# Kudo510/ImageSequenceRegistrationfor6DPoseEstimationLabeling

Measured on AMD Instinct MI355X. Metric: registered images/sec (T-LESS obj 1-like, synthetic) + final Chamfer error, higher is better.
Workload: dtype bf16

## Files before the change

imagesequenceregistrationfor6dposeestimationlabeling_amd/_capi.py:

```python
from __future__ import annotations

import ctypes as C
from pathlib import Path

import torch

import os

_PKG = Path(__file__).resolve().parent
LIB_PATH = Path(os.environ["ISR_HIP_LIB"]) if os.environ.get("ISR_HIP_LIB") else _PKG / "libisr_hip.so"

ISR_OK = 0
ABI_VERSION = 6
DTYPE_BF16 = 0
DTYPE_F32 = 1
DTYPE_BF16_LOG2 = 2
DTYPE_BF16_LOG2_SCREENED = 3
RANSAC_STAGED = 0
RANSAC_SEQUENTIAL = 1
INLIERS_REFIT = 0
INLIERS_RANSAC = 1
FINAL_REFIT = 0
FINAL_EPNP = 1
TUNE = {"nn_path": 0, "nn_filter": 1, "icp_warm": 2, "nn_plan_rq": 3, "nn_plan_blocks": 4,
        "nn_tile_st": 5, "nn_tile_sq": 6, "nn_tile_tb": 7, "ep_wsum_valu": 8, "k1_f32_chain": 9, "k1_split": 10}


class IsrError(RuntimeError):
    pass


_lib = None

_vp = C.c_void_p
_i = C.c_int
_sz = C.c_size_t
_d = C.c_double
_f = C.c_float
_u64 = C.c_uint64
_i64 = C.c_int64

SIGNATURES = {
    "isr_abi_version": (_i, []),
    "isr_last_error": (C.c_char_p, []),
    "isr_device_count": (_i, []),
    "isr_tuning_set": (_i, [_i, _i]),
    "isr_tuning_get": (_i, [_i]),
    "isr_corr_argmax_workspace_bytes": (_sz, [_i, _i, _i, _i]),
# ... 91 lines not shown
DENSITY_SIGNATURES = {
    "isr_density_pack_bytes": (_sz, [_i, _vp, _i]),
    "isr_density_pack": (_i, [_i, _vp, _i, _vp, _f, _vp, _vp, _vp, _sz]),
    "isr_density_eval": (_i, [_vp, _sz, _i, _vp, _i, _vp, _i, _vp, _vp]),
    "isr_density_march": (_i, [_vp, _sz, _i, _vp, _i, _vp, _vp, _vp, _i, _i, _f, _vp, _vp, _vp, _vp, _vp, _vp]),
    "isr_density_eval_host": (_i, [_vp, _sz, _i, _vp, _i, _vp, _i, _vp]),
    "isr_density_march_host": (_i, [_vp, _sz, _i, _vp, _i, _vp, _vp, _vp, _i, _i, _f, _vp, _vp, _vp, _vp, _vp]),
    "isr_density_sincos_host": (_i, [_vp, _sz, _vp, _vp]),
    "isr_density_activations_host": (_i, [_vp, _sz, _f, _vp, _vp]),
}

DENSITY_DIR_SIGNATURES = {
    "isr_density_march_dir": (_i, [_vp, _sz, _i, _vp, _i, _vp, _vp, _vp, _i, _i, _f, _i, _vp, _vp, _vp, _vp, _vp, _vp]),
    "isr_density_march_dir_host": (_i, [_vp, _sz, _i, _vp, _i, _vp, _vp, _vp, _i, _i, _f, _i, _vp, _vp, _vp, _vp, _vp]),
    "isr_density_march_given_host": (_i, [_vp, _vp, _i, _i, _f, _i, _vp, _vp, _vp]),
}

RADIUS_SIGNATURES = {
    "isr_radius_workspace_bytes": (_sz, [_i]),
    "isr_radius_count": (_i, [_vp, _i, _d, _i, _vp, _vp, _sz, _vp]),
    "isr_radius_count_host": (_i, [_vp, _i, _d, _i, _vp]),
}

KNN_SIGNATURES = {
    "isr_knn_workspace_bytes": (_sz, [_i, _i, _i]),
    "isr_knn": (_i, [_vp, _i, _vp, _i, _i, _vp, _vp, _vp, _sz, _vp]),
    "isr_knn_host": (_i, [_vp, _i, _vp, _i, _i, _vp, _vp]),
    "isr_local_frames": (_i, [_vp, _i, _vp, _i, _i, _vp, _vp, _vp]),
    "isr_local_frames_host": (_i, [_vp, _i, _vp, _i, _i, _vp, _vp]),
}

_RAYS_SPEC = [_i, _vp, _vp, _vp, _vp, _i, _i, _i, _i, _i, _f, _f, _f, _f, _f, _f, _i, _u64]
RAYS_SIGNATURES = {
    "isr_rays_workspace_bytes": (_sz, [_i, _i]),
    "isr_rays_bundle": (_i, [*_RAYS_SPEC, _vp, _vp, _vp, _vp, _vp]),
    "isr_rays_bundle_host": (_i, [*_RAYS_SPEC, _vp, _vp, _vp, _vp]),
    "isr_rays_select_count": (_i, [*_RAYS_SPEC, _vp, _i, _i, _vp, _vp, _sz, _vp]),
    "isr_rays_select_emit": (_i, [*_RAYS_SPEC, _vp, _i, _i, _vp, _sz, _i64, _vp, _vp, _vp, _vp, _vp, _vp]),
    "isr_rays_select_count_host": (_i, [*_RAYS_SPEC, _vp, _i, _i, _vp]),
    "isr_rays_select_emit_host": (_i, [*_RAYS_SPEC, _vp, _i, _i, _i64, _vp, _vp, _vp, _vp, _vp]),
    "isr_sample_nearest": (_i, [_vp, _i, _i, _i, _i, _vp, _i, _vp, _vp]),
    "isr_sample_nearest_host": (_i, [_vp, _i, _i, _i, _i, _vp, _i, _vp]),
    "isr_rays_philox_host": (_i, [_vp, _vp, _vp, _vp]),
}

_RADIANCE_FIELD = [_vp, _sz, _i, _vp, _i, _i, _i]
# ... 144 lines not shown
    "isr_seq_refit_sums_host": (_i, [_vp, _vp, _vp, _vp, _vp, _vp, _i, _i, _i, _d, _vp, _vp, _vp]),
}


def lib() -> C.CDLL:
    global _lib
    if _lib is not None:
        return _lib
    if not LIB_PATH.exists():
        raise IsrError(
            f"{LIB_PATH} is missing: build it with "
            "`python -m imagesequenceregistrationfor6dposeestimationlabeling_amd.build` "
            "(there is no CPU fallback)")
    try:
        L = C.CDLL(str(LIB_PATH))
    except OSError as e:
        raise IsrError(f"cannot load {LIB_PATH}: {e}") from e
    for name, (res, args) in {**SIGNATURES, **FIELD_SIGNATURES, **FPS_SIGNATURES, **DENSITY_SIGNATURES,
                               **DENSITY_DIR_SIGNATURES, **RADIUS_SIGNATURES, **MC_SIGNATURES, **KNN_SIGNATURES,
                               **RAYS_SIGNATURES, **RADIANCE_SIGNATURES, **RESAMPLE_SIGNATURES,
                               **CONTRASTIVE_SIGNATURES, **FIELD_GRAD_SIGNATURES, **SAMPLE_GRAD_SIGNATURES,
                               **EA_GRAD_SIGNATURES, **RADIANCE_GRAD_SIGNATURES, **AUGMENT_SIGNATURES,
                               **ADAM_SIGNATURES, **RAY_LOSSES_SIGNATURES, **COLOR_AUG_SIGNATURES, **INGEST_SIGNATURES,
                               **ICP_PLANE_SIGNATURES, **SEQ_REFIT_SIGNATURES}.items():
        try:
            fn = getattr(L, name)
        except AttributeError as e:
            raise IsrError(f"{LIB_PATH} does not export {name}") from e
        fn.restype = res
        fn.argtypes = args
    if L.isr_abi_version() != ABI_VERSION:
        raise IsrError(f"ABI version {L.isr_abi_version()} != {ABI_VERSION}")
    _lib = L
    return L


def check(rc: int, what: str) -> None:
    if rc != ISR_OK:
        msg = lib().isr_last_error()
        raise IsrError(f"{what} failed ({rc}): {msg.decode() if msg else ''}")


def ptr(t) -> int | None:
    if t is None:
        return None
    return t.data_ptr()

# ... 22 lines not shown
```

imagesequenceregistrationfor6dposeestimationlabeling_amd/csrc/capi_common.hip:

```cpp
#include "isr_common.hpp"

#include <atomic>
#include <cstdlib>
#include <cstring>

namespace isr {

char* last_error_buf() {
  static thread_local char buf[512] = {0};
  return buf;
}

void set_error(const char* fmt, ...) {
  va_list ap;
  va_start(ap, fmt);
  vsnprintf(last_error_buf(), 512, fmt, ap);
  va_end(ap);
}

namespace {

struct Tuning {
  std::atomic<int> v[ISR_TUNE_COUNT];
  Tuning() {
    const int defaults[ISR_TUNE_COUNT] = {-1, -1, 1, 0, 0, 0, 0, 0, 0, 0, 0};
    for (int i = 0; i < ISR_TUNE_COUNT; ++i) v[i].store(defaults[i], std::memory_order_relaxed);
    if (const char* e = getenv("ISR_NN_GRID")) { if (e[0] >= '0' && e[0] <= '2') v[ISR_TUNE_NN_PATH] = e[0] - '0'; }
    if (const char* e = getenv("ISR_NN_FILTER")) { if (e[0] == '0' || e[0] == '1') v[ISR_TUNE_NN_FILTER] = e[0] - '0'; }
    if (const char* e = getenv("ISR_ICP_WARM")) { if (e[0] == '0') v[ISR_TUNE_ICP_WARM] = 0; }
    if (const char* e = getenv("ISR_NN_PLAN")) {
      int rq = 0; long want = 0;
      if (sscanf(e, "%d,%ld", &rq, &want) >= 1) {
        if (rq == 1 || rq == 4) v[ISR_TUNE_NN_PLAN_RQ] = rq;
        if (want > 0) v[ISR_TUNE_NN_PLAN_BLOCKS] = (int)want;
      }
    }
    if (const char* e = getenv("ISR_NN_TILE")) {
      double st = 0, sq = 0; int tb = 0;
      (void)sscanf(e, "%lf,%lf,%d", &st, &sq, &tb);
      if (st > 0) v[ISR_TUNE_NN_TILE_ST] = (int)(st * 1000.0 + 0.5);
      if (sq > 0) v[ISR_TUNE_NN_TILE_SQ] = (int)(sq * 1000.0 + 0.5);
      if (tb > 0) v[ISR_TUNE_NN_TILE_TB] = tb;
    }
  }
};

Tuning& tuning_state() {
  static Tuning t;
  return t;
}

const int tuning_loaded = (tuning_state(), 0);
// ... 85 lines not shown
```

imagesequenceregistrationfor6dposeestimationlabeling_amd/csrc/nn_batched.hip:

```cpp
#include "block_prims.hpp"
#include "isr_common.hpp"

#include <cstddef>
#include <cstdlib>

namespace {

#ifndef ISR_NN_PACKED_BATCH
#define ISR_NN_PACKED_BATCH 1
#endif
constexpr int kThreads = 256;
constexpr int kTile = 256;
constexpr int kGroup = 8;
constexpr int kNV = 18;

__device__ __forceinline__ void xform64(const double* __restrict__ T, float x, float y, float z,
                                        double& ox, double& oy, double& oz) {
  if (T == nullptr) {
    ox = x; oy = y; oz = z;
    return;
  }
  const double dx = x, dy = y, dz = z;
  ox = fma(T[2], dz, fma(T[1], dy, fma(T[0], dx, T[3])));
  oy = fma(T[6], dz, fma(T[5], dy, fma(T[4], dx, T[7])));
  oz = fma(T[10], dz, fma(T[9], dy, fma(T[8], dx, T[11])));
}

constexpr int kUnresolved = -2;

template <int RQ>
__device__ __forceinline__ int query_of(int r) {
  return (int)blockIdx.x * RQ * kThreads + ((int)threadIdx.x >> 6) * (RQ * 64) + r * 64 + ((int)threadIdx.x & 63);
}

__global__ __launch_bounds__(256) void tile_box_kernel(const float* __restrict__ tgt, int Nt, float* __restrict__ box) {
  __shared__ float red[6][4];
  const int j = blockIdx.x * 256 + threadIdx.x;
  float v[6] = {3.0e38f, 3.0e38f, 3.0e38f, -3.0e38f, -3.0e38f, -3.0e38f};
  if (j < Nt) {
#pragma unroll
    for (int a = 0; a < 3; ++a) v[a] = v[3 + a] = tgt[3 * (size_t)j + a];
  }
#pragma unroll
  for (int a = 0; a < 3; ++a) {
#pragma unroll
    for (int o = 32; o >= 1; o >>= 1) {
      v[a] = fminf(v[a], __shfl_xor(v[a], o, 64));
      v[3 + a] = fmaxf(v[3 + a], __shfl_xor(v[3 + a], o, 64));
    }
  }
  if ((threadIdx.x & 63) == 0) {
// ... 846 lines not shown
      launch_search(p, grid, stream, qry, Nq, tgt, Nt, tq, tt, packed ? nullptr : part_d2, packed ? nullptr : part_idx, nullptr, unres,
                    packed, nullptr);
    ISR_CHECK_LAUNCH("nn_search_kernel");
    const dim3 fgrid(p.fblocks, nb);
    if (cov)
      nn_finalize_kernel<true><<<fgrid, kThreads, 0, stream>>>(qry, Nq, tgt, Tq, Tt, p.nsplit,
                                                               radius, part_d2, part_idx, b0,
                                                               nn_idx, nn_d, part_sums, nullptr, packed);
    else
      nn_finalize_kernel<false><<<fgrid, kThreads, 0, stream>>>(qry, Nq, tgt, Tq, Tt, p.nsplit,
                                                                radius, part_d2, part_idx, b0,
                                                                nn_idx, nn_d, part_sums, nullptr, packed);
    ISR_CHECK_LAUNCH("nn_finalize_kernel");
  }
  if (sum_d || sum_d2 || n_in || cov) {
    const dim3 rblock(32, 8);
    nn_reduce_kernel<<<(B + 7) / 8, rblock, 0, stream>>>(part_sums, p.fblocks, B, sum_d, sum_d2,
                                                         n_in, cov);
    ISR_CHECK_LAUNCH("nn_reduce_kernel");
  }
  return ISR_OK;
}

extern "C" int isr_add_metric(const float* verts, int V, const double* Ta, const double* Tb, int B,
                              double* mean_out, isr_stream_t stream) {
  ISR_REQUIRE(verts && mean_out, "isr_add_metric: null pointer");
  ISR_REQUIRE(V > 0 && B > 0, "isr_add_metric: V=%d B=%d", V, B);
  add_metric_kernel<<<B, kThreads, 0, isr::as_stream(stream)>>>(verts, V, Ta, Tb, mean_out);
  ISR_CHECK_LAUNCH("add_metric_kernel");
  return ISR_OK;
}

extern "C" size_t isr_icp_workspace_bytes(int Ns, int Nt) {
  if (Ns <= 0 || Nt <= 0) return 0;
  const NNPlan p = make_plan(Ns, Nt, 1, true);
  return isr::align_up((size_t)p.fblocks * kNV * sizeof(double), 256) + isr::align_up((size_t)Ns * 8, 256) +
         2 * isr::align_up((size_t)Ns * 4, 256) + isr::align_up((size_t)((Nt + kTile - 1) / kTile) * 6 * sizeof(float), 256) + 2048;
}

extern "C" int isr_icp_point_to_point(const float* src, int Ns, const float* tgt, int Nt, double threshold,
                                      int max_iter, double rel_fitness, double rel_rmse, double* T_io,
                                      double* result, void* ws, size_t ws_bytes, isr_stream_t stream_) {
  ISR_REQUIRE(src && tgt && T_io && result, "isr_icp_point_to_point: null pointer");
  ISR_REQUIRE(Ns > 0 && Nt > 0 && max_iter >= 0 && threshold > 0, "isr_icp_point_to_point: Ns=%d Nt=%d max_iter=%d", Ns, Nt, max_iter);
  if (!ws || ws_bytes < isr_icp_workspace_bytes(Ns, Nt)) {
    isr::set_error("isr_icp_point_to_point: workspace %zu < %zu", ws_bytes, isr_icp_workspace_bytes(Ns, Nt));
// ... 319 lines not shown
```

imagesequenceregistrationfor6dposeestimationlabeling_amd/ops.py:

```python
from __future__ import annotations

import ctypes
from dataclasses import dataclass
from typing import NamedTuple

import numpy as np

import torch

from . import _capi
from ._capi import check, current_stream, lib, ptr, require_cuda

_workspaces: dict[tuple, torch.Tensor] = {}

_timers: dict[str, list] | None = None


def enable_timing(on: bool = True) -> None:
    global _timers
    _timers = {} if on else None


def drain_timing() -> dict[str, tuple[int, float, float]]:
    out = {}
    if _timers is None:
# ... 101 lines not shown
        if T is not None:
            if T.numel() % 12:
                raise ValueError("transforms must be (B,3,4)")
            B = max(B, T.numel() // 12)
    for T in (Tq, Tt):
        if T is not None and T.numel() // 12 != B:
            raise ValueError("Tq and Tt must have the same batch size")
    Nq, Nt = qry.shape[0], tgt.shape[0]
    L = lib()
    sum_d = torch.empty(B, dtype=torch.float64, device=dev)
    sum_d2 = torch.empty(B, dtype=torch.float64, device=dev)
    n_in = torch.empty(B, dtype=torch.int32, device=dev)
    nn_idx = torch.empty((B, Nq), dtype=torch.int32, device=dev) if want_idx else None
    nn_d = torch.empty((B, Nq), dtype=torch.float64, device=dev) if want_dist else None
    cov = torch.empty((B, 16), dtype=torch.float64, device=dev) if want_cov else None
    nbytes = L.isr_nn_batched_workspace_bytes(Nq, Nt, B)
    ws = workspace(dev, nbytes, "nn")
    with torch.cuda.device(dev), _timed("nn_batched", float(B) * Nq * Nt):
        rc = L.isr_nn_batched(ptr(qry), Nq, ptr(tgt), Nt, ptr(Tq), ptr(Tt), B, float(radius),
                              ptr(sum_d), ptr(sum_d2), ptr(n_in), ptr(nn_idx), ptr(nn_d), ptr(cov),
                              ptr(ws), ws.numel(), current_stream(dev))
    check(rc, "isr_nn_batched")
    return NNResult(sum_d, sum_d2, n_in, nn_idx, nn_d, cov)


def icp_point_to_point_batch(sources: torch.Tensor, target: torch.Tensor, state: torch.Tensor, threshold: float,
                             max_iter: int = 30, rel_fitness: float = 1e-6, rel_rmse: float = 1e-6) -> torch.Tensor:
    dev = require_cuda(sources, target, state)
    if sources.dtype != torch.float32 or target.dtype != torch.float32 or not (sources.is_contiguous() and target.is_contiguous()):
        raise ValueError("icp_point_to_point_batch: sources and target must be contiguous float32")
    if state.dtype != torch.float64 or state.ndim != 2 or state.shape[1] != 20 or not state.is_contiguous():
        raise ValueError(f"icp_point_to_point_batch: state must be contiguous (B,20) float64, got {tuple(state.shape)} {state.dtype}")
    if target.ndim != 2 or target.shape[1] != 3 or sources.ndim not in (2, 3) or sources.shape[-1] != 3:
        raise ValueError(f"icp_point_to_point_batch: sources {tuple(sources.shape)} must be (Ns,3) or (B,Ns,3), target "
                         f"{tuple(target.shape)} (Nt,3)")
    B, Ns, Nt = state.shape[0], sources.shape[-2], target.shape[0]
    if sources.ndim == 3 and sources.shape[0] != B:
        raise ValueError(f"icp_point_to_point_batch: sources {tuple(sources.shape)} and state {tuple(state.shape)} disagree on B")
    stride = 3 * Ns if sources.ndim == 3 else 0
    L = lib()
    ws = workspace(dev, L.isr_icp_point_to_point_batch_workspace_bytes(Ns, Nt, B), "icp")
    with torch.cuda.device(dev), _timed("icp_batch", float(B) * Ns * Nt * (max_iter + 1)):
        rc = L.isr_icp_point_to_point_batch(ptr(sources), stride, Ns, ptr(target), Nt, B, float(threshold), int(max_iter),
                                            float(rel_fitness), float(rel_rmse), ptr(state), ptr(ws), ws.numel(),
                                            current_stream(dev))
    check(rc, "isr_icp_point_to_point_batch")
# ... 2553 lines not shown
```

imagesequenceregistrationfor6dposeestimationlabeling_amd/registration.py:

```python
from __future__ import annotations

import numpy as np
import torch

from . import ops
from ._capi import IsrError

SOLVEPNP_P3P = 2
SOLVEPNP_AP3P = 5

_state = {"surface_pts": None, "device": None}


def device() -> torch.device:
    if not torch.cuda.is_available():
        raise IsrError("no HIP device visible: the registration hot path has no CPU fallback")
    return torch.device("cuda", torch.cuda.current_device())


def _dev(x, dtype=None) -> torch.Tensor:
    if isinstance(x, torch.Tensor):
        t = x if x.is_cuda else x.to(device())
    else:
        t = torch.from_numpy(np.ascontiguousarray(x)).to(device())
# ... 115 lines not shown

def vote_error_rows(model_verts, surface_pts, gt_rel, pred_rel, diameter, chunk=4096):
    v, sp = _dev(model_verts, torch.float32), _dev(surface_pts, torch.float32)
    g = np.asarray(gt_rel, np.float64)[..., :3, :].reshape(-1, 12)
    p = np.asarray(pred_rel, np.float64)[..., :3, :].reshape(-1, 12)
    rows, n = np.asarray(gt_rel).shape[:2]
    adds = np.empty(rows * n)
    for s in range(0, rows * n, chunk):
        r = ops.nn_batched(v, sp, _dev(g[s:s + chunk]), _dev(p[s:s + chunk]))
        adds[s:s + chunk] = (r.sum_d / v.shape[0]).cpu().numpy()
    adds = adds.reshape(rows, n)
    return (adds < 0.1 * diameter).astype(np.float64), adds


def choose_image(error, top=50):
    s = np.sum(error, axis=1)
    return int(np.argmax(s)), np.argsort(-s, kind="stable")[:top]


def chamfer(pc_a, pc_b, Ta=None, Tb=None):
    a, b = _dev(pc_a, torch.float32), _dev(pc_b, torch.float32)
    ta = None if Ta is None else _dev(np.asarray(Ta, np.float64).reshape(1, 12))
    tb = None if Tb is None else _dev(np.asarray(Tb, np.float64).reshape(1, 12))
    ab = ops.nn_batched(a, b, ta, tb)
    ba = ops.nn_batched(b, a, tb, ta)
    return 0.5 * (float(ab.sum_d.item()) / a.shape[0] + float(ba.sum_d.item()) / b.shape[0])


def chamfer_pairs(pc1, R_pred, R_rel_gt):
    pc = _dev(pc1, torch.float32)
    Rp = np.asarray(R_pred, np.float64)
    Rr = np.asarray(R_rel_gt, np.float64)
    n1 = Rp.shape[0] - 1
    Tg = np.zeros((n1, 3, 4))
    Tp = np.zeros((n1, 3, 4))
    Tg[:, :, :3] = np.einsum("nji,njk->nik", Rr, Rp[:-1])
    Tp[:, :, :3] = np.transpose(Rp[1:], (0, 2, 1))
    tg, tp = _dev(Tg.reshape(n1, 12)), _dev(Tp.reshape(n1, 12))
    ab = ops.nn_batched(pc, pc, tp, tg)
    ba = ops.nn_batched(pc, pc, tg, tp)
    return 0.5 * (ab.sum_d + ba.sum_d) / pc.shape[0]


def choose_best(chamferdis):
    c = chamferdis.cpu().numpy() if isinstance(chamferdis, torch.Tensor) else np.asarray(chamferdis)
    i = int(np.argmin(c))
    return i, float(c[i])


def _eval(src, tgt, threshold, T):
    dev = src.device
    Tq = torch.from_numpy(np.ascontiguousarray(np.asarray(T, np.float64)[:3, :].reshape(1, 12))).to(dev)
    buf = torch.empty(18, dtype=torch.float64, device=dev)
    Nq, Nt = src.shape[0], tgt.shape[0]
    L = ops.lib()
    ws = ops.workspace(dev, L.isr_nn_batched_workspace_bytes(Nq, Nt, 1), "nn")
    base = buf.data_ptr()
    with torch.cuda.device(dev):
        rc = L.isr_nn_batched(ops.ptr(src), Nq, ops.ptr(tgt), Nt, ops.ptr(Tq), None, 1, float(threshold), base, base + 8,
                              None, None, None, base + 16, ops.ptr(ws), ws.numel(), ops.current_stream(dev))
# ... 222 lines not shown
```

include/isr_hip.h:

```cpp
#ifndef ISR_HIP_H
#define ISR_HIP_H

#include <stddef.h>
#include <stdint.h>

#ifdef __cplusplus
extern "C" {
#endif

#define ISR_ABI_VERSION 6

#define ISR_OK 0
#define ISR_ERR_ARG (-1)
#define ISR_ERR_WORKSPACE (-2)
#define ISR_ERR_HIP (-3)
#define ISR_ERR_UNSUPPORTED (-4)

#define ISR_DTYPE_BF16 0
#define ISR_DTYPE_F32 1
#define ISR_DTYPE_BF16_LOG2 2

#define ISR_DTYPE_BF16_LOG2_SCREENED 3

typedef void* isr_stream_t;

int isr_abi_version(void);
const char* isr_last_error(void);
int isr_device_count(void);

#define ISR_TUNE_NN_PATH 0
#define ISR_TUNE_NN_FILTER 1
#define ISR_TUNE_ICP_WARM 2
#define ISR_TUNE_NN_PLAN_RQ 3
#define ISR_TUNE_NN_PLAN_BLOCKS 4
#define ISR_TUNE_NN_TILE_ST 5
#define ISR_TUNE_NN_TILE_SQ 6
#define ISR_TUNE_NN_TILE_TB 7
#define ISR_TUNE_EP_WSUM_VALU 8
#define ISR_TUNE_K1_F32_CHAIN 9
#define ISR_TUNE_K1_SPLIT 10
#define ISR_TUNE_COUNT 11
int isr_tuning_set(int knob, int value);
int isr_tuning_get(int knob);

size_t isr_corr_argmax_workspace_bytes(int P, int N, int D, int dtype);
int isr_corr_argmax(const void* Q, const void* K, int P, int N, int D, int ldq, int ldk, int dtype,
                    int32_t* idx, float* logp, float* lse, void* ws, size_t ws_bytes,
                    isr_stream_t stream);

int isr_corr_argmax_digits(const void* Q, const void* K, int P, int N, int D, int ldq, int ldk, int dtype,
                           int32_t* idx, float* logp, float* lse, int rows_per_image, const int32_t* n_rows,
                           int32_t* digit_hist, void* ws, size_t ws_bytes, isr_stream_t stream);

int isr_corr_argmax_phase(const void* Q, const void* K, int P, int N, int D, int ldq, int ldk, int dtype,
                          int32_t* idx, float* logp, float* lse, int rows_per_image, const int32_t* n_rows,
                          int32_t* digit_hist, int phase, void* ws, size_t ws_bytes, isr_stream_t stream);

int isr_corr_argmax_recheck_count(const void* ws, size_t ws_bytes, int P, int N, int dtype,
                                  int32_t* count_host, isr_stream_t stream);
int isr_corr_argmax_recheck_count_f32(const void* ws, size_t ws_bytes, int P, int N, int D, int32_t* count_host,
                                      isr_stream_t stream);

int isr_corr_quantize_fp6(const void* X, int R, int ld, void* out, float* nrm, float* kmax, isr_stream_t stream);

// ... 188 lines not shown
```

Before: 1126.

## Add certified self-cloud nearest-neighbour path using precomputed kNN table for chamfer

Adds a path for nearest-neighbour queries where the query and target are the same cloud under two nearby rigid transforms. A per-cloud kNN table and a max-radius bound are built and cached. A first kernel tries to certify each point's nearest neighbour from its table neighbours, and only uncertified points fall through to the existing brute-force search. Chamfer and chamfer_pairs route near transform pairs through this path by default. The cost is a table build and kNN precompute per cloud, plus Python-side splitting by transform pairs, and the saving depends on how many points are certified.

```diff
diff --git a/imagesequenceregistrationfor6dposeestimationlabeling_amd/_capi.py b/imagesequenceregistrationfor6dposeestimationlabeling_amd/_capi.py
--- a/imagesequenceregistrationfor6dposeestimationlabeling_amd/_capi.py
+++ b/imagesequenceregistrationfor6dposeestimationlabeling_amd/_capi.py
@@ -23,7 +23,7 @@
 FINAL_REFIT = 0
 FINAL_EPNP = 1
 TUNE = {"nn_path": 0, "nn_filter": 1, "icp_warm": 2, "nn_plan_rq": 3, "nn_plan_blocks": 4,
-        "nn_tile_st": 5, "nn_tile_sq": 6, "nn_tile_tb": 7, "ep_wsum_valu": 8, "k1_f32_chain": 9, "k1_split": 10}
+        "nn_tile_st": 5, "nn_tile_sq": 6, "nn_tile_tb": 7, "ep_wsum_valu": 8, "k1_f32_chain": 9, "k1_split": 10, "nn_self": 11}
 
 
 class IsrError(RuntimeError):
@@ -161,6 +161,16 @@
     "isr_radius_count_host": (_i, [_vp, _i, _d, _i, _vp]),
 }
 
+NN_SELF_SIGNATURES = {
+    "isr_nn_self_table_bytes": (_sz, [_i, _i]),
+    "isr_nn_self_table_build_workspace_bytes": (_sz, [_i, _i]),
+    "isr_nn_self_table_build": (_i, [_vp, _i, _i, _vp, _vp, _sz, _vp]),
+    "isr_nn_self_table_build_host": (_i, [_vp, _i, _i, _vp]),
+    "isr_nn_batched_self_workspace_bytes": (_sz, [_i, _i]),
+    "isr_nn_batched_self": (_i, [_vp, _i, _vp, _i, _vp, _vp, _i, _d, _vp, _vp, _vp, _vp, _vp, _vp, _vp, _sz, _vp]),
+    "isr_nn_batched_self_host": (_i, [_vp, _i, _vp, _i, _vp, _vp, _i, _vp, _vp, _vp]),
+}
+
 KNN_SIGNATURES = {
     "isr_knn_workspace_bytes": (_sz, [_i, _i, _i]),
     "isr_knn": (_i, [_vp, _i, _vp, _i, _i, _vp, _vp, _vp, _sz, _vp]),
@@ -351,7 +361,7 @@
                                **CONTRASTIVE_SIGNATURES, **FIELD_GRAD_SIGNATURES, **SAMPLE_GRAD_SIGNATURES,
                                **EA_GRAD_SIGNATURES, **RADIANCE_GRAD_SIGNATURES, **AUGMENT_SIGNATURES,
                                **ADAM_SIGNATURES, **RAY_LOSSES_SIGNATURES, **COLOR_AUG_SIGNATURES, **INGEST_SIGNATURES,
-                               **ICP_PLANE_SIGNATURES, **SEQ_REFIT_SIGNATURES}.items():
+                               **ICP_PLANE_SIGNATURES, **SEQ_REFIT_SIGNATURES, **NN_SELF_SIGNATURES}.items():
         try:
             fn = getattr(L, name)
         except AttributeError as e:
diff --git a/imagesequenceregistrationfor6dposeestimationlabeling_amd/csrc/capi_common.hip b/imagesequenceregistrationfor6dposeestimationlabeling_amd/csrc/capi_common.hip
--- a/imagesequenceregistrationfor6dposeestimationlabeling_amd/csrc/capi_common.hip
+++ b/imagesequenceregistrationfor6dposeestimationlabeling_amd/csrc/capi_common.hip
@@ -23,11 +23,12 @@
 struct Tuning {
   std::atomic<int> v[ISR_TUNE_COUNT];
   Tuning() {
-    const int defaults[ISR_TUNE_COUNT] = {-1, -1, 1, 0, 0, 0, 0, 0, 0, 0, 0};
+    const int defaults[ISR_TUNE_COUNT] = {-1, -1, 1, 0, 0, 0, 0, 0, 0, 0, 0, 1};
     for (int i = 0; i < ISR_TUNE_COUNT; ++i) v[i].store(defaults[i], std::memory_order_relaxed);
     if (const char* e = getenv("ISR_NN_GRID")) { if (e[0] >= '0' && e[0] <= '2') v[ISR_TUNE_NN_PATH] = e[0] - '0'; }
     if (const char* e = getenv("ISR_NN_FILTER")) { if (e[0] == '0' || e[0] == '1') v[ISR_TUNE_NN_FILTER] = e[0] - '0'; }
     if (const char* e = getenv("ISR_ICP_WARM")) { if (e[0] == '0') v[ISR_TUNE_ICP_WARM] = 0; }
+    if (const char* e = getenv("ISR_NN_SELF")) { if (e[0] == '0') v[ISR_TUNE_NN_SELF] = 0; }
     if (const char* e = getenv("ISR_NN_PLAN")) {
       int rq = 0; long want = 0;
       if (sscanf(e, "%d,%ld", &rq, &want) >= 1) {
diff --git a/imagesequenceregistrationfor6dposeestimationlabeling_amd/csrc/nn_batched.hip b/imagesequenceregistrationfor6dposeestimationlabeling_amd/csrc/nn_batched.hip
--- a/imagesequenceregistrationfor6dposeestimationlabeling_amd/csrc/nn_batched.hip
+++ b/imagesequenceregistrationfor6dposeestimationlabeling_amd/csrc/nn_batched.hip
@@ -1,5 +1,8 @@
 #include "block_prims.hpp"
 #include "isr_common.hpp"
+#include "nn_self.hpp"
+
+#include "../../include/isr_nn_self.h"
 
 #include <cstddef>
 #include <cstdlib>
@@ -27,6 +30,7 @@
 }
 
 constexpr int kUnresolved = -2;
+static_assert(kUnresolved == isr::nnself::kUnresolvedIdx, "nn_self.hpp names the same mark");
 
 template <int RQ>
 __device__ __forceinline__ int query_of(int r) {
@@ -919,6 +923,101 @@
   return ISR_OK;
 }
 
+namespace {
+
+__global__ __launch_bounds__(kThreads) void nn_self_kernel(const float* __restrict__ cloud, int N,
+                                                           const int32_t* __restrict__ tab_idx,
+                                                           const float* __restrict__ tab_d2, const float* __restrict__ rmax2,
+                                                           int K, const double* __restrict__ Tq, const double* __restrict__ Tt,
+                                                           float* __restrict__ part_d2, int32_t* __restrict__ part_idx,
+                                                           int32_t* __restrict__ unresolved) {
+  const int b = blockIdx.y;
+  const int i = blockIdx.x * kThreads + threadIdx.x;
+  const double* tq = Tq ? Tq + 12 * (size_t)b : nullptr;
+  const double* tt = Tt ? Tt + 12 * (size_t)b : nullptr;
+  const isr::nnself::ItemBound ib = isr::nnself::item_bound(tt, *rmax2);
+  bool open = false;
+  if (i < N) {
+    const isr::nnself::SelfResult r =
+        isr::nnself::self_query(cloud, N, tab_idx + (size_t)i * K, tab_d2 + (size_t)i * K, K, i, tq, tt, ib);
+    const size_t o = (size_t)b * N + i;
+    part_d2[o] = r.certified ? r.best : __builtin_inff();
+    part_idx[o] = r.certified ? r.idx : kUnresolved;
+    open = !r.certified;
+  }
+  const unsigned long long m = __ballot(open);
+  if (m != 0 && (threadIdx.x & 63) == 0) atomicAdd(unresolved, (int32_t)__popcll(m));
+}
+
+NNPlan make_self_plan(int N, int B) {
+  NNPlan p = make_plan(N, N, B, true);
+  p.nsplit = 1;
+  p.split_len = ((N + kTile - 1) / kTile) * kTile;
+  long bc = (long)(kPartBudget / ((size_t)N * 8));
+  if (bc < 1) bc = 1;
+  if (bc > B) bc = B;
+  if (bc > 65535) bc = 65535;
+  p.bchunk = (int)bc;
+  return p;
+}
+
+}
+
+extern "C" size_t isr_nn_batched_self_workspace_bytes(int N, int B) {
+  if (N <= 0 || B <= 0) return 0;
+  const NNPlan p = make_self_plan(N, B);
+  return 256 + 2 * isr::align_up((size_t)p.bchunk * N * 4, 256) + isr::align_up((size_t)B * p.fblocks * kNV * sizeof(double), 256) +
+         256;
+}
+
+extern "C" int isr_nn_batched_self(const float* cloud, int N, const void* table, int K, const double* Tq, const double* Tt,
+                                   int B, double radius, double* sum_d, double* sum_d2, int32_t* n_in, int32_t* nn_idx,
+                                   double* nn_d, double* cov, void* ws, size_t ws_bytes, isr_stream_t stream_) {
+  ISR_REQUIRE(cloud && table, "isr_nn_batched_self: null pointer");
+  ISR_REQUIRE(N > 0 && N <= (1 << 24) && B > 0, "isr_nn_batched_self: N=%d (1..2^24) B=%d must be positive", N, B);
+  ISR_REQUIRE(K >= 1 && K <= isr::nnself::kMaxK, "isr_nn_batched_self: K = %d (1..%d)", K, isr::nnself::kMaxK);
+  ISR_REQUIRE(sum_d || sum_d2 || n_in || nn_idx || nn_d || cov, "isr_nn_batched_self: no output requested");
+  if (!ws || ws_bytes < isr_nn_batched_self_workspace_bytes(N, B)) {
+    isr::set_error("isr_nn_batched_self: workspace %zu < %zu", ws_bytes, isr_nn_batched_self_workspace_bytes(N, B));
+    return ISR_ERR_WORKSPACE;
+  }
+  hipStream_t stream = isr::as_stream(stream_);
+  const NNPlan p = make_self_plan(N, B);
+  isr::Workspace w(ws, ws_bytes);
+  int32_t* unresolved = w.take<int32_t>(64);
+  float* part_d2 = w.take<float>((size_t)p.bchunk * N);
+  int32_t* part_idx = w.take<int32_t>((size_t)p.bchunk * N);
+  double* part_sums = w.take<double>((size_t)B * p.fblocks * kNV);
+  ISR_CHECK_HIP(hipMemsetAsync(unresolved, 0, 256, stream));
+  const int32_t* tab_idx = isr::nnself::table_idx(table);
+  const float* tab_d2 = isr::nnself::table_d2(table, N, K);
+  const float* rmax2 = isr::nnself::table_rmax2(table, N, K);
+  for (int b0 = 0; b0 < B; b0 += p.bchunk) {
+    const int nb = (B - b0 < p.bchunk) ? (B - b0) : p.bchunk;
+    const double* tq = Tq ? Tq + 12 * (size_t)b0 : nullptr;
+    const double* tt = Tt ? Tt + 12 * (size_t)b0 : nullptr;
+    nn_self_kernel<<<dim3(p.fblocks, nb), kThreads, 0, stream>>>(cloud, N, tab_idx, tab_d2, rmax2, K, tq, tt, part_d2, part_idx,
+                                                                 unresolved);
+    ISR_CHECK_LAUNCH("nn_self_kernel");
+    launch_search(p, dim3(p.qblocks, 1, nb), stream, cloud, N, cloud, N, tq, tt, part_d2, part_idx, nullptr, unresolved, nullptr,
+                  nullptr);
+    ISR_CHECK_LAUNCH("nn_search_kernel");
+    const dim3 fgrid(p.fblocks, nb);
+    if (cov)
+      nn_finalize_kernel<true><<<fgrid, kThreads, 0, stream>>>(cloud, N, cloud, Tq, Tt, 1, radius, part_d2, part_idx, b0, nn_idx,
+                                                               nn_d, part_sums, nullptr, nullptr);
+    else
+      nn_finalize_kernel<false><<<fgrid, kThreads, 0, stream>>>(cloud, N, cloud, Tq, Tt, 1, radius, part_d2, part_idx, b0, nn_idx,
+                                                                nn_d, part_sums, nullptr, nullptr);
+    ISR_CHECK_LAUNCH("nn_finalize_kernel");
+  }
+  if (sum_d || sum_d2 || n_in || cov) {
+    nn_reduce_kernel<<<(B + 7) / 8, dim3(32, 8), 0, stream>>>(part_sums, p.fblocks, B, sum_d, sum_d2, n_in, cov);
+    ISR_CHECK_LAUNCH("nn_reduce_kernel");
+  }
+  return ISR_OK;
+}
+
 extern "C" int isr_add_metric(const float* verts, int V, const double* Ta, const double* Tb, int B,
                               double* mean_out, isr_stream_t stream) {
   ISR_REQUIRE(verts && mean_out, "isr_add_metric: null pointer");
diff --git a/imagesequenceregistrationfor6dposeestimationlabeling_amd/csrc/nn_self.hip b/imagesequenceregistrationfor6dposeestimationlabeling_amd/csrc/nn_self.hip
--- /dev/null
+++ b/imagesequenceregistrationfor6dposeestimationlabeling_amd/csrc/nn_self.hip
@@ -0,0 +1,147 @@
+#include "nn_self.hpp"
+#include "isr_common.hpp"
+
+#include "../../include/isr_knn.h"
+#include "../../include/isr_nn_self.h"
+
+#include <vector>
+
+namespace {
+
+using namespace isr::nnself;
+
+constexpr int kThreads = 256;
+
+int knn_width(int N, int K) { return N < K + 1 ? N : K + 1; }
+
+__global__ __launch_bounds__(kThreads) void self_table_pack_kernel(const int32_t* __restrict__ knn_idx,
+                                                                   const float* __restrict__ knn_d2, int N, int Kk, int K,
+                                                                   int32_t* __restrict__ idx, float* __restrict__ d2) {
+  const long i = (long)blockIdx.x * kThreads + threadIdx.x;
+  if (i >= N) return;
+  pack_row(knn_idx + (size_t)i * Kk, knn_d2 + (size_t)i * Kk, Kk, K, (int)i, idx + (size_t)i * K, d2 + (size_t)i * K);
+}
+
+__global__ __launch_bounds__(kThreads) void self_table_rmax2_kernel(const float* __restrict__ cloud, int N,
+                                                                    float* __restrict__ out) {
+  __shared__ float red[kThreads / 64];
+  float m = 0.f;
+  for (int j = threadIdx.x; j < N; j += kThreads) {
+    const float x = cloud[3 * (size_t)j], y = cloud[3 * (size_t)j + 1], z = cloud[3 * (size_t)j + 2];
+    m = fmaxf(m, __builtin_fmaf(z, z, __builtin_fmaf(y, y, x * x)));
+  }
+#pragma unroll
+  for (int o = 32; o >= 1; o >>= 1) m = fmaxf(m, __shfl_xor(m, o, 64));
+  if ((threadIdx.x & 63) == 0) red[threadIdx.x >> 6] = m;
+  __syncthreads();
+  if (threadIdx.x == 0) *out = 1.0001f * fmaxf(fmaxf(red[0], red[1]), fmaxf(red[2], red[3]));
+}
+
+int check_table_shape(const char* who, int N, int K) {
+  ISR_REQUIRE(N >= 1 && N <= (1 << 24), "%s: N = %d (1..2^24)", who, N);
+  ISR_REQUIRE(K >= 1 && K <= kMaxK, "%s: K = %d (1..%d)", who, K, kMaxK);
+  return ISR_OK;
+}
+
+}
+
+extern "C" size_t isr_nn_self_table_bytes(int N, int K) {
+  if (check_table_shape("isr_nn_self_table_bytes", N, K)) return 0;
+  return table_bytes(N, K);
+}
+
+extern "C" size_t isr_nn_self_table_build_workspace_bytes(int N, int K) {
+  if (check_table_shape("isr_nn_self_table_build_workspace_bytes", N, K)) return 0;
+  const int Kk = knn_width(N, K);
+  return isr::align_up(isr_knn_workspace_bytes(N, N, Kk), 256) + 2 * isr::align_up((size_t)N * Kk * 4, 256) + 256;
+}
+
+extern "C" int isr_nn_self_table_build(const float* cloud, int N, int K, void* table, void* ws, size_t ws_bytes,
+                                       isr_stream_t stream_) {
+  if (int rc = check_table_shape("isr_nn_self_table_build", N, K)) return rc;
+  ISR_REQUIRE(cloud && table, "isr_nn_self_table_build: null pointer");
+  if (!ws || ws_bytes < isr_nn_self_table_build_workspace_bytes(N, K)) {
+    isr::set_error("isr_nn_self_table_build: workspace %zu < %zu", ws_bytes, isr_nn_self_table_build_workspace_bytes(N, K));
+    return ISR_ERR_WORKSPACE;
+  }
+  hipStream_t stream = isr::as_stream(stream_);
+  const int Kk = knn_width(N, K);
+  isr::Workspace w(ws, ws_bytes);
+  const size_t knn_ws = isr_knn_workspace_bytes(N, N, Kk);
+  char* kws = w.take<char>(knn_ws);
+  int32_t* kidx = w.take<int32_t>((size_t)N * Kk);
+  float* kd2 = w.take<float>((size_t)N * Kk);
+  if (int rc = isr_knn(cloud, N, cloud, N, Kk, kidx, kd2, kws, knn_ws, stream_)) return rc;
+  char* t = static_cast<char*>(table);
+  const unsigned blocks = (unsigned)(((long)N + kThreads - 1) / kThreads);
+  self_table_pack_kernel<<<blocks, kThreads, 0, stream>>>(kidx, kd2, N, Kk, K, reinterpret_cast<int32_t*>(t),
+                                                          reinterpret_cast<float*>(t + table_part_bytes(N, K)));
+  ISR_CHECK_LAUNCH("self_table_pack_kernel");
+  self_table_rmax2_kernel<<<1, kThreads, 0, stream>>>(cloud, N, reinterpret_cast<float*>(t + 2 * table_part_bytes(N, K)));
+  ISR_CHECK_LAUNCH("self_table_rmax2_kernel");
+  return ISR_OK;
+}
+
+extern "C" int isr_nn_self_table_build_host(const float* cloud, int N, int K, void* table) {
+  if (int rc = check_table_shape("isr_nn_self_table_build_host", N, K)) return rc;
+  ISR_REQUIRE(cloud && table, "isr_nn_self_table_build_host: null pointer");
+  const int Kk = knn_width(N, K);
+  std::vector<int32_t> kidx((size_t)N * Kk);
+  std::vector<float> kd2((size_t)N * Kk);
+  if (int rc = isr_knn_host(cloud, N, cloud, N, Kk, kidx.data(), kd2.data())) return rc;
+  char* t = static_cast<char*>(table);
+  int32_t* idx = reinterpret_cast<int32_t*>(t);
+  float* d2 = reinterpret_cast<float*>(t + table_part_bytes(N, K));
+  float m = 0.f;
+  for (int i = 0; i < N; ++i) {
+    pack_row(kidx.data() + (size_t)i * Kk, kd2.data() + (size_t)i * Kk, Kk, K, i, idx + (size_t)i * K, d2 + (size_t)i * K);
+    const float x = cloud[3 * (size_t)i], y = cloud[3 * (size_t)i + 1], z = cloud[3 * (size_t)i + 2];
+    m = fmaxf(m, fmaf(z, z, fmaf(y, y, x * x)));
+  }
+  *reinterpret_cast<float*>(t + 2 * table_part_bytes(N, K)) = 1.0001f * m;
+  return ISR_OK;
+}
+
+extern "C" int isr_nn_batched_self_host(const float* cloud, int N, const void* table, int K, const double* Tq, const double* Tt,
+                                        int B, int32_t* nn_idx, float* d2, uint8_t* certified) {
+  if (int rc = check_table_shape("isr_nn_batched_self_host", N, K)) return rc;
+  ISR_REQUIRE(cloud && table, "isr_nn_batched_self_host: null pointer");
+  ISR_REQUIRE(B > 0, "isr_nn_batched_self_host: B = %d must be positive", B);
+  const int32_t* tidx = table_idx(table);
+  const float* td2 = table_d2(table, N, K);
+  const float rmax2 = *table_rmax2(table, N, K);
+  for (int b = 0; b < B; ++b) {
+    const double* tq = Tq ? Tq + 12 * (size_t)b : nullptr;
+    const double* tt = Tt ? Tt + 12 * (size_t)b : nullptr;
+    const ItemBound ib = item_bound(tt, rmax2);
+    std::vector<float> t((size_t)3 * N);
+    bool have_t = false;
+    for (int i = 0; i < N; ++i) {
+      SelfResult r = self_query(cloud, N, tidx + (size_t)i * K, td2 + (size_t)i * K, K, i, tq, tt, ib);
+      if (!r.certified) {
+        double x, y, z;
+        if (!have_t) {
+          for (int j = 0; j < N; ++j) {
+            xform(tt, cloud[3 * (size_t)j], cloud[3 * (size_t)j + 1], cloud[3 * (size_t)j + 2], x, y, z);
+            t[3 * (size_t)j] = (float)x; t[3 * (size_t)j + 1] = (float)y; t[3 * (size_t)j + 2] = (float)z;
+          }
+          have_t = true;
+        }
+        xform(tq, cloud[3 * (size_t)i], cloud[3 * (size_t)i + 1], cloud[3 * (size_t)i + 2], x, y, z);
+        const float qx = (float)x, qy = (float)y, qz = (float)z;
+        r.best = inf32();
+        r.idx = -1;
+        for (int j = 0; j < N; ++j) {
+          const float dx = qx - t[3 * (size_t)j], dy = qy - t[3 * (size_t)j + 1], dz = qz - t[3 * (size_t)j + 2];
+          const float d = fmaf(dz, dz, fmaf(dy, dy, dx * dx));
+          if (d < r.best) { r.best = d; r.idx = j; }
+        }
+      }
+      const size_t o = (size_t)b * N + i;
+      if (nn_idx) nn_idx[o] = r.idx;
+      if (d2) d2[o] = r.best;
+      if (certified) certified[o] = r.certified ? 1 : 0;
+    }
+  }
+  return ISR_OK;
+}
diff --git a/imagesequenceregistrationfor6dposeestimationlabeling_amd/csrc/nn_self.hpp b/imagesequenceregistrationfor6dposeestimationlabeling_amd/csrc/nn_self.hpp
--- /dev/null
+++ b/imagesequenceregistrationfor6dposeestimationlabeling_amd/csrc/nn_self.hpp
@@ -0,0 +1,119 @@
+#pragma once
+#include <cmath>
+#include <cstddef>
+#include <cstdint>
+
+#include "hd.hpp"
+
+namespace isr {
+namespace nnself {
+
+constexpr int kMaxK = 32;
+constexpr int kUnresolvedIdx = -2;
+constexpr double kU = 5.9604644775390625e-08;
+constexpr double kEtaMax = 1e-3;
+
+ISR_HD size_t table_part_bytes(int N, int K) { return ((size_t)N * K * 4 + 255) / 256 * 256; }
+ISR_HD size_t table_bytes(int N, int K) { return 2 * table_part_bytes(N, K) + 256; }
+ISR_HD const int32_t* table_idx(const void* table) { return static_cast<const int32_t*>(table); }
+ISR_HD const float* table_d2(const void* table, int N, int K) {
+  return reinterpret_cast<const float*>(static_cast<const char*>(table) + table_part_bytes(N, K));
+}
+ISR_HD const float* table_rmax2(const void* table, int N, int K) {
+  return reinterpret_cast<const float*>(static_cast<const char*>(table) + 2 * table_part_bytes(N, K));
+}
+
+ISR_HD float inf32() { return bits_float(0x7F800000u); }
+
+ISR_HD void pack_row(const int32_t* knn_idx, const float* knn_d2, int Kk, int K, int i, int32_t* idx, float* d2) {
+  int w = 0;
+  for (int r = 0; r < Kk && w < K; ++r) {
+    if (knn_idx[r] == i) continue;
+    idx[w] = knn_idx[r];
+    d2[w] = knn_d2[r];
+    ++w;
+  }
+  for (; w < K; ++w) {
+    idx[w] = -1;
+    d2[w] = inf32();
+  }
+}
+
+ISR_HD void xform(const double* T, float x, float y, float z, double& ox, double& oy, double& oz) {
+  if (T == nullptr) {
+    ox = x; oy = y; oz = z;
+    return;
+  }
+  const double dx = x, dy = y, dz = z;
+  ox = fma(T[2], dz, fma(T[1], dy, fma(T[0], dx, T[3])));
+  oy = fma(T[6], dz, fma(T[5], dy, fma(T[4], dx, T[7])));
+  oz = fma(T[10], dz, fma(T[9], dy, fma(T[8], dx, T[11])));
+}
+
+struct ItemBound {
+  double one_minus_eta, dt;
+  bool ok;
+};
+
+ISR_HD ItemBound item_bound(const double* Tt, float rmax2) {
+  ItemBound ib;
+  double eta = 0.0, tn = 0.0;
+  if (Tt != nullptr) {
+    double s = 0.0;
+    for (int a = 0; a < 3; ++a)
+      for (int c = 0; c < 3; ++c) {
+        const double m = fma(Tt[8 + a], Tt[8 + c], fma(Tt[4 + a], Tt[4 + c], Tt[a] * Tt[c])) - (a == c ? 1.0 : 0.0);
+        s = fma(m, m, s);
+      }
+    eta = sqrt(s) + 1e-12;
+    tn = sqrt(fma(Tt[11], Tt[11], fma(Tt[7], Tt[7], Tt[3] * Tt[3])));
+  }
+  const double tmax = 1.001 * ((1.0 + eta) * sqrt((double)rmax2) + tn) + 1e-18;
+  ib.one_minus_eta = 1.0 - eta;
+  ib.dt = 2.002 * kU * tmax;
+  ib.ok = eta < kEtaMax && tmax < 1.0e300;
+  return ib;
+}
+
+struct SelfResult {
+  float best;
+  int32_t idx;
+  bool certified;
+};
+
+ISR_HD SelfResult self_query(const float* cloud, int N, const int32_t* row, const float* row_d2, int K, int i, const double* tq,
+                             const double* tt, const ItemBound& ib) {
+  double x, y, z;
+  xform(tq, cloud[3 * (size_t)i], cloud[3 * (size_t)i + 1], cloud[3 * (size_t)i + 2], x, y, z);
+  const float qx = (float)x, qy = (float)y, qz = (float)z;
+  SelfResult r;
+  r.best = inf32();
+  r.idx = -1;
+  float dii = 0.f;
+  for (int c = -1; c < K; ++c) {
+    const int j = c < 0 ? i : row[c];
+    if (j < 0 || j >= N || (c >= 0 && j == i)) continue;
+    xform(tt, cloud[3 * (size_t)j], cloud[3 * (size_t)j + 1], cloud[3 * (size_t)j + 2], x, y, z);
+    const float dx = qx - (float)x, dy = qy - (float)y, dz = qz - (float)z;
+    const float d = fmaf(dz, dz, fmaf(dy, dy, dx * dx));
+    if (c < 0) dii = d;
+    const bool up = (d < r.best) | ((d == r.best) & (j < r.idx));
+    r.best = up ? d : r.best;
+    r.idx = up ? j : r.idx;
+  }
+  const float g = row_d2[K - 1];
+  bool cert = ib.ok & (r.idx >= 0) & (dii < inf32());
+  if (!(g == inf32())) {
+    const double G2 = (double)g * (1.0 - 8.0 * kU) - 1e-37;
+    const double G = G2 > 0.0 ? sqrt(G2) : 0.0;
+    const double E = sqrt((double)dii * (1.0 + 8.0 * kU) + 1e-37);
+    const double Y = ib.one_minus_eta * G - E - ib.dt;
+    const double LB = (Y * Y * (1.0 - 8.0 * kU) - 1e-37) * (1.0 - 1e-9);
+    cert = cert & (Y > 0.0) & (LB > (double)r.best);
+  }
+  r.certified = cert;
+  return r;
+}
+
+}
+}
diff --git a/imagesequenceregistrationfor6dposeestimationlabeling_amd/ops.py b/imagesequenceregistrationfor6dposeestimationlabeling_amd/ops.py
--- a/imagesequenceregistrationfor6dposeestimationlabeling_amd/ops.py
+++ b/imagesequenceregistrationfor6dposeestimationlabeling_amd/ops.py
@@ -1,6 +1,8 @@
 from __future__ import annotations
 
 import ctypes
+import threading
+import weakref
 from dataclasses import dataclass
 from typing import NamedTuple
 
@@ -148,6 +150,155 @@
                               ptr(ws), ws.numel(), current_stream(dev))
     check(rc, "isr_nn_batched")
     return NNResult(sum_d, sum_d2, n_in, nn_idx, nn_d, cov)
+
+
+NN_SELF_K = 8
+
+
+@dataclass
+class NNSelfTable:
+    table: torch.Tensor
+    N: int
+    K: int
+    event: torch.cuda.Event
+    stream: int
+    rmax: float
+    g_low: float
+
+    def wait(self, dev: torch.device) -> None:
+        cur = torch.cuda.current_stream(dev)
+        if cur.cuda_stream != self.stream:
+            cur.wait_event(self.event)
+            self.table.record_stream(cur)
+
+
+_self_tables: dict[tuple, NNSelfTable] = {}
+_self_memo: list = [None]
+_self_lock = threading.Lock()
+_self_last: list = [None]
+
+
+def _self_key(cloud: torch.Tensor) -> tuple:
+    memo = _self_memo[0]
+    if memo is not None and memo[0]() is cloud and memo[1] == cloud._version:
+        return memo[2]
+    from .sequence import cloud_key
+    key = cloud_key(cloud)
+    _self_memo[0] = (weakref.ref(cloud), cloud._version, key)
+    return key
+
+
+def nn_self_table(cloud: torch.Tensor, K: int = NN_SELF_K) -> NNSelfTable:
+    dev = require_cuda(cloud)
+    if cloud.dtype != torch.float32 or cloud.ndim != 2 or cloud.shape[1] != 3 or not cloud.is_contiguous():
+        raise ValueError(f"nn_self_table: cloud must be contiguous (N,3) float32, got {tuple(cloud.shape)} {cloud.dtype}")
+    with _self_lock:
+        key = _self_key(cloud) + (int(K),)
+        tab = _self_tables.get(key)
+        if tab is None:
+            if len(_self_tables) > 4:
+                _self_tables.clear()
+            N, L = cloud.shape[0], lib()
+            nbytes = L.isr_nn_self_table_bytes(N, K)
+            if nbytes == 0:
+                raise _capi.IsrError(L.isr_last_error().decode())
+            table = torch.empty(nbytes, dtype=torch.uint8, device=dev)
+            ws = torch.empty(L.isr_nn_self_table_build_workspace_bytes(N, K), dtype=torch.uint8, device=dev)
+            with torch.cuda.device(dev):
+                rc = L.isr_nn_self_table_build(ptr(cloud), N, K, ptr(table), ptr(ws), ws.numel(), current_stream(dev))
+                check(rc, "isr_nn_self_table_build")
+                ev = torch.cuda.Event()
+                ev.record()
+                part = (N * K * 4 + 255) // 256 * 256
+                g = table[part:part + N * K * 4].view(torch.float32).view(N, K)[:, K - 1]
+                hdr = table[2 * part:2 * part + 4].view(torch.float32)
+                stats = torch.cat([g.kthvalue(max(1, N // 20)).values.reshape(1), hdr]).sqrt().cpu().numpy()
+            tab = _self_tables[key] = NNSelfTable(table, N, int(K), ev, torch.cuda.current_stream(dev).cuda_stream,
+                                                  float(stats[1]), float(stats[0]))
+    return tab
+
+
+def nn_batched_self(cloud: torch.Tensor, Tq: torch.Tensor | None = None, Tt: torch.Tensor | None = None,
+                    radius: float = -1.0, want_idx: bool = False, want_dist: bool = False, want_cov: bool = False,
+                    table: NNSelfTable | None = None) -> NNResult:
+    dev = require_cuda(cloud, Tq, Tt)
+    cloud, Tq, Tt = _f32c(cloud), _f64c(Tq), _f64c(Tt)
+    if cloud.ndim != 2 or cloud.shape[1] != 3:
+        raise ValueError(f"cloud must be (N,3): got {tuple(cloud.shape)}")
+    B = 1
+    for T in (Tq, Tt):
+        if T is not None:
+            if T.numel() % 12:
+                raise ValueError("transforms must be (B,3,4)")
+            B = max(B, T.numel() // 12)
+    for T in (Tq, Tt):
+        if T is not None and T.numel() // 12 != B:
+            raise ValueError("Tq and Tt must have the same batch size")
+    N = cloud.shape[0]
+    tab = table if table is not None else nn_self_table(cloud)
+    if tab.N != N:
+        raise ValueError(f"nn_batched_self: the table is of a cloud of {tab.N} points, this one has {N}")
+    tab.wait(dev)
+    L = lib()
+    sum_d = torch.empty(B, dtype=torch.float64, device=dev)
+    sum_d2 = torch.empty(B, dtype=torch.float64, device=dev)
+    n_in = torch.empty(B, dtype=torch.int32, device=dev)
+    nn_idx = torch.empty((B, N), dtype=torch.int32, device=dev) if want_idx else None
+    nn_d = torch.empty((B, N), dtype=torch.float64, device=dev) if want_dist else None
+    cov = torch.empty((B, 16), dtype=torch.float64, device=dev) if want_cov else None
+    ws = workspace(dev, L.isr_nn_batched_self_workspace_bytes(N, B), "nn_self")
+    with torch.cuda.device(dev), _timed("nn_batched_self", float(B) * N * (tab.K + 1)):
+        rc = L.isr_nn_batched_self(ptr(cloud), N, ptr(tab.table), tab.K, ptr(Tq), ptr(Tt), B, float(radius),
+                                   ptr(sum_d), ptr(sum_d2), ptr(n_in), ptr(nn_idx), ptr(nn_d), ptr(cov),
+                                   ptr(ws), ws.numel(), current_stream(dev))
+    check(rc, "isr_nn_batched_self")
+    _self_last[0] = (ws, B * N)
+    return NNResult(sum_d, sum_d2, n_in, nn_idx, nn_d, cov)
+
+
+def nn_self_last_uncertified() -> tuple[int, int] | None:
+    last = _self_last[0]
+    if last is None:
+        return None
+    torch.cuda.synchronize()
+    return int(last[0][:4].view(torch.int32).item()), last[1]
+
+
+NN_SELF_NEAR = 0.45
+
+
+def nn_self_near(tab: NNSelfTable, Ta: np.ndarray, Tb: np.ndarray) -> np.ndarray:
+    Ta, Tb = np.asarray(Ta, np.float64).reshape(-1, 3, 4), np.asarray(Tb, np.float64).reshape(-1, 3, 4)
+    with np.errstate(invalid="ignore", over="ignore"):
+        disp = np.linalg.norm(Ta[:, :, :3] - Tb[:, :, :3], axis=(1, 2)) * tab.rmax + np.linalg.norm(Ta[:, :, 3] - Tb[:, :, 3], axis=1)
+        return disp <= NN_SELF_NEAR * tab.g_low
+
+
+def nn_self_enabled() -> bool:
+    return lib().isr_tuning_get(_capi.TUNE["nn_self"]) != 0
+
+
+def nn_self_table_host(cloud, K: int = NN_SELF_K) -> np.ndarray:
+    c = np.ascontiguousarray(cloud, np.float32)
+    L = lib()
+    table = np.zeros(L.isr_nn_self_table_bytes(c.shape[0], K), np.uint8)
+    check(L.isr_nn_self_table_build_host(c.ctypes.data, c.shape[0], K, table.ctypes.data), "isr_nn_self_table_build_host")
+    return table
+
+
+def nn_batched_self_host(cloud, table: np.ndarray, Tq=None, Tt=None, K: int = NN_SELF_K):
+    c = np.ascontiguousarray(cloud, np.float32)
+    N = c.shape[0]
+    tq = None if Tq is None else np.ascontiguousarray(Tq, np.float64).reshape(-1, 12)
+    tt = None if Tt is None else np.ascontiguousarray(Tt, np.float64).reshape(-1, 12)
+    B = max([1] + [t.shape[0] for t in (tq, tt) if t is not None])
+    idx = np.empty((B, N), np.int32)
+    d2 = np.empty((B, N), np.float32)
+    cert = np.empty((B, N), np.uint8)
+    hp = lambda a: None if a is None else a.ctypes.data
+    check(lib().isr_nn_batched_self_host(hp(c), N, hp(table), K, hp(tq), hp(tt), B, hp(idx), hp(d2), hp(cert)),
+          "isr_nn_batched_self_host")
+    return idx, d2, cert.astype(bool)
 
 
 def icp_point_to_point_batch(sources: torch.Tensor, target: torch.Tensor, state: torch.Tensor, threshold: float,
diff --git a/imagesequenceregistrationfor6dposeestimationlabeling_amd/registration.py b/imagesequenceregistrationfor6dposeestimationlabeling_amd/registration.py
--- a/imagesequenceregistrationfor6dposeestimationlabeling_amd/registration.py
+++ b/imagesequenceregistrationfor6dposeestimationlabeling_amd/registration.py
@@ -161,9 +161,34 @@
     a, b = _dev(pc_a, torch.float32), _dev(pc_b, torch.float32)
     ta = None if Ta is None else _dev(np.asarray(Ta, np.float64).reshape(1, 12))
     tb = None if Tb is None else _dev(np.asarray(Tb, np.float64).reshape(1, 12))
+    if a is b and Ta is not None and Tb is not None and ops.nn_self_enabled():
+        ab_sum, ba_sum = _same_cloud_sums(a, np.asarray(Ta, np.float64).reshape(1, 12), np.asarray(Tb, np.float64).reshape(1, 12))
+        return 0.5 * (float(ab_sum.item()) + float(ba_sum.item())) / a.shape[0]
     ab = ops.nn_batched(a, b, ta, tb)
     ba = ops.nn_batched(b, a, tb, ta)
     return 0.5 * (float(ab.sum_d.item()) / a.shape[0] + float(ba.sum_d.item()) / b.shape[0])
+
+
+def _same_cloud_sums(pc: torch.Tensor, Ta: np.ndarray, Tb: np.ndarray):
+    pc = pc.contiguous()
+    tab = ops.nn_self_table(pc)
+    near = ops.nn_self_near(tab, Ta, Tb)
+    B = Ta.shape[0]
+    out = [torch.empty(B, dtype=torch.float64, device=pc.device) for _ in range(2)]
+    for sel, self_route in ((near, True), (~near, False)):
+        if not sel.any():
+            continue
+        ta, tb = _dev(np.ascontiguousarray(Ta[sel])), _dev(np.ascontiguousarray(Tb[sel]))
+        if self_route:
+            ab, ba = ops.nn_batched_self(pc, ta, tb, table=tab), ops.nn_batched_self(pc, tb, ta, table=tab)
+        else:
+            ab, ba = ops.nn_batched(pc, pc, ta, tb), ops.nn_batched(pc, pc, tb, ta)
+        if sel.all():
+            return ab.sum_d, ba.sum_d
+        where = torch.from_numpy(np.flatnonzero(sel)).to(pc.device)
+        out[0][where] = ab.sum_d
+        out[1][where] = ba.sum_d
+    return out[0], out[1]
 
 
 def chamfer_pairs(pc1, R_pred, R_rel_gt):
@@ -175,6 +200,9 @@
     Tp = np.zeros((n1, 3, 4))
     Tg[:, :, :3] = np.einsum("nji,njk->nik", Rr, Rp[:-1])
     Tp[:, :, :3] = np.transpose(Rp[1:], (0, 2, 1))
+    if n1 > 0 and ops.nn_self_enabled():
+        ab_sum, ba_sum = _same_cloud_sums(pc, Tp.reshape(n1, 12), Tg.reshape(n1, 12))
+        return 0.5 * (ab_sum + ba_sum) / pc.shape[0]
     tg, tp = _dev(Tg.reshape(n1, 12)), _dev(Tp.reshape(n1, 12))
     ab = ops.nn_batched(pc, pc, tp, tg)
     ba = ops.nn_batched(pc, pc, tg, tp)
diff --git a/include/isr_hip.h b/include/isr_hip.h
--- a/include/isr_hip.h
+++ b/include/isr_hip.h
@@ -39,7 +39,8 @@
 #define ISR_TUNE_EP_WSUM_VALU 8
 #define ISR_TUNE_K1_F32_CHAIN 9
 #define ISR_TUNE_K1_SPLIT 10
-#define ISR_TUNE_COUNT 11
+#define ISR_TUNE_NN_SELF 11
+#define ISR_TUNE_COUNT 12
 int isr_tuning_set(int knob, int value);
 int isr_tuning_get(int knob);
 
diff --git a/include/isr_nn_self.h b/include/isr_nn_self.h
--- /dev/null
+++ b/include/isr_nn_self.h
@@ -0,0 +1,28 @@
+#ifndef ISR_NN_SELF_H
+#define ISR_NN_SELF_H
+
+#include <stddef.h>
+#include <stdint.h>
+
+#include "isr_hip.h"
+
+#ifdef __cplusplus
+extern "C" {
+#endif
+
+size_t isr_nn_self_table_bytes(int N, int K);
+size_t isr_nn_self_table_build_workspace_bytes(int N, int K);
+int isr_nn_self_table_build(const float* cloud, int N, int K, void* table, void* ws, size_t ws_bytes, isr_stream_t stream);
+int isr_nn_self_table_build_host(const float* cloud, int N, int K, void* table);
+size_t isr_nn_batched_self_workspace_bytes(int N, int B);
+int isr_nn_batched_self(const float* cloud, int N, const void* table, int K, const double* Tq, const double* Tt, int B,
+                        double radius, double* sum_d, double* sum_d2, int32_t* n_in, int32_t* nn_idx, double* nn_d,
+                        double* cov, void* ws, size_t ws_bytes, isr_stream_t stream);
+int isr_nn_batched_self_host(const float* cloud, int N, const void* table, int K, const double* Tq, const double* Tt, int B,
+                             int32_t* nn_idx, float* d2, uint8_t* certified);
+
+#ifdef __cplusplus
+}
+#endif
+
+#endif
```

Result: no change. 1125 (-0.1%).
